# pallgeuer/novic

Measured on NVIDIA B200. Metric: labels/sec (greedy, batch 4096), higher is better.
Workload: dtype bf16

## Files before the change

include/novic_b200.h:

```cpp
#ifndef NOVIC_B200_H_
#define NOVIC_B200_H_

#include <stddef.h>
#include <stdint.h>

#ifdef __cplusplus
extern "C" {
#endif

#define NOVIC_MAX_LAYERS 16
#define NOVIC_MAX_BEAMS 16

typedef struct NovicCfg {
  int32_t embed_dim;
  int32_t hidden_dim;
  int32_t ffn_dim;
  int32_t num_layers;
  int32_t num_heads;
  int32_t prefix_len;
  int32_t vocab_size;
  int32_t token_length;
  int32_t strictly_causal;
  int32_t num_end_loss;
  float ln_eps;
// ... 157 lines not shown
  const float* proj_w[NOVIC_VIT_MAX_LAYERS];
  const float* proj_b[NOVIC_VIT_MAX_LAYERS];
  const float* norm2_w[NOVIC_VIT_MAX_LAYERS];
  const float* norm2_b[NOVIC_VIT_MAX_LAYERS];
  const float* fc1_w[NOVIC_VIT_MAX_LAYERS];
  const float* fc1_b[NOVIC_VIT_MAX_LAYERS];
  const float* fc2_w[NOVIC_VIT_MAX_LAYERS];
  const float* fc2_b[NOVIC_VIT_MAX_LAYERS];
} NovicSiglipWeights;
int novic_siglip_create(const NovicSiglipCfg* cfg, NovicVitHandle** out);
int novic_siglip_set_weights(NovicVitHandle* h, const NovicSiglipWeights* w, void* wbuf, size_t wbuf_bytes, void* stream);

int novic_debug_gemm(const void* a_bf16, const void* w_bf16, float* out, int32_t M, int32_t N, int32_t K,
                     int32_t block_n, void* stream);

int novic_debug_transpose_bf16(const void* src, int64_t rows, int32_t cols, int32_t ld_src, void* dst, int32_t ld_dst, void* stream);
int novic_debug_wgrad(const void* a_t, int32_t Mo, const void* b_t, int32_t No, int64_t K, int32_t ld, float* dw, void* stream);
int novic_debug_wgrad_mn(const void* a, int32_t Mo, int32_t ld_a, const void* b, int32_t No, int32_t ld_b, int64_t K, float* dw, void* stream);
int32_t novic_debug_wgrad_splits(int64_t tiles, int64_t kblocks, int32_t sms);

int novic_debug_vit_gemm(const void* a, const void* w, int32_t M, int32_t N, int32_t K, int32_t epi, int32_t act, int32_t direct, const float* bias,
                         void* dst, int32_t ld, const float* table, int32_t patches, int32_t tok0, int32_t path, int32_t grid_div, void* stream);
int novic_debug_vit_attention(const void* qkv, int32_t nimg, int32_t T, int32_t W, int32_t heads, int32_t kernel, int32_t max_ctas, void* out, void* stream);
int novic_debug_siglip_map_attention(const void* kv, const float* q, int32_t nimg, int32_t T, int32_t W, int32_t heads, void* out, void* stream);
int novic_debug_vit_layernorm(float* x, int64_t in_stride, const float* w1, const float* b1, const float* w2, const float* b2, int32_t store_x, void* out_bf,
                              int32_t rows, int32_t W, float eps, const float* cls, const float* pos0, int32_t cls_period, void* stream);

int novic_kernel_timing(int32_t enable);
int novic_kernel_times(double* ms_out, int64_t* count_out, int32_t n_classes);

// ... 20 lines not shown
```

novic_b200/_abi.py:

```python
from __future__ import annotations

import ctypes as C
import os
import subprocess

NOVIC_MAX_LAYERS = 16
NOVIC_MAX_BEAMS = 16

_HERE = os.path.dirname(os.path.abspath(__file__))
LIB_PATH = os.path.join(_HERE, "lib", "libnovic_b200.so")
CSRC_DIR = os.path.join(_HERE, "csrc")


class NovicCfg(C.Structure):
    _fields_ = [
        ("embed_dim", C.c_int32), ("hidden_dim", C.c_int32), ("ffn_dim", C.c_int32), ("num_layers", C.c_int32),
        ("num_heads", C.c_int32), ("prefix_len", C.c_int32), ("vocab_size", C.c_int32), ("token_length", C.c_int32),
        ("strictly_causal", C.c_int32), ("num_end_loss", C.c_int32), ("ln_eps", C.c_float), ("label_smoothing", C.c_float),
    ]


_FP = C.c_void_p


# ... 78 lines not shown
                                         C.c_void_p, C.c_size_t, C.c_void_p, C.c_int32, C.c_void_p]),
    "novic_adamw_scratch_bytes": (C.c_size_t, []),
    "novic_adamw_step": (C.c_int, [C.POINTER(NovicAdamW), _FP, _FP, _FP, _FP, C.c_int64, _FP, _FP, C.c_void_p, C.c_size_t, _FP, C.c_void_p]),
    "novic_vit_create": (C.c_int, [C.POINTER(NovicVitCfg), C.POINTER(C.c_void_p)]),
    "novic_vit_destroy": (C.c_int, [C.c_void_p]),
    "novic_vit_weight_bytes": (C.c_size_t, [C.c_void_p]),
    "novic_vit_set_weights": (C.c_int, [C.c_void_p, C.POINTER(NovicVitWeights), C.c_void_p, C.c_size_t, C.c_void_p]),
    "novic_vit_workspace_bytes": (C.c_size_t, [C.c_void_p, C.c_int64]),
    "novic_vit_encode": (C.c_int, [C.c_void_p, _FP, C.c_int64, _FP, C.c_int32, C.c_int64, C.c_void_p, C.c_size_t, C.c_void_p]),
    "novic_siglip_create": (C.c_int, [C.POINTER(NovicSiglipCfg), C.POINTER(C.c_void_p)]),
    "novic_siglip_set_weights": (C.c_int, [C.c_void_p, C.POINTER(NovicSiglipWeights), C.c_void_p, C.c_size_t, C.c_void_p]),
    "novic_set_dropout": (C.c_int, [C.c_void_p, C.c_float, C.c_float, C.c_uint64]),
    "novic_noise_apply": (C.c_int, [C.POINTER(NovicNoiseCfg), _FP, C.c_int64, C.c_uint64, C.c_uint64, C.c_void_p]),
    "novic_noise_apply_predrawn": (C.c_int, [C.POINTER(NovicNoiseCfg), _FP, C.c_int64, _FP, _FP, _FP, _FP, C.c_void_p]),
    "novic_debug_gemm": (C.c_int, [_FP, _FP, _FP, C.c_int32, C.c_int32, C.c_int32, C.c_int32, C.c_void_p]),
    "novic_debug_trace": (C.c_int, [C.POINTER(C.c_int64), C.c_int32]),
    "novic_debug_ws_offset": (C.c_int, [C.c_void_p, C.c_int64, C.c_int32, C.c_int32, C.c_char_p, C.POINTER(C.c_size_t)]),
    "novic_debug_keep_classes": (C.c_int, [C.c_void_p, C.c_uint32]),
    "novic_debug_redzone": (C.c_int, [C.c_size_t]),
    "novic_debug_zones": (C.c_int64, [C.c_void_p, C.c_int32, C.c_int64, C.c_int32, C.c_int32, C.POINTER(C.c_uint64), C.c_int64]),
    "novic_debug_transpose_bf16": (C.c_int, [_FP, C.c_int64, C.c_int32, C.c_int32, _FP, C.c_int32, C.c_void_p]),
    "novic_debug_wgrad": (C.c_int, [_FP, C.c_int32, _FP, C.c_int32, C.c_int64, C.c_int32, _FP, C.c_void_p]),
    "novic_debug_wgrad_mn": (C.c_int, [_FP, C.c_int32, C.c_int32, _FP, C.c_int32, C.c_int32, C.c_int64, _FP, C.c_void_p]),
    "novic_debug_wgrad_splits": (C.c_int32, [C.c_int64, C.c_int64, C.c_int32]),
    "novic_debug_vit_gemm": (C.c_int, [_FP, _FP, C.c_int32, C.c_int32, C.c_int32, C.c_int32, C.c_int32, C.c_int32, _FP, _FP, C.c_int32, _FP,
                                       C.c_int32, C.c_int32, C.c_int32, C.c_int32, C.c_void_p]),
    "novic_debug_vit_attention": (C.c_int, [_FP, C.c_int32, C.c_int32, C.c_int32, C.c_int32, C.c_int32, C.c_int32, _FP, C.c_void_p]),
    "novic_debug_siglip_map_attention": (C.c_int, [_FP, _FP, C.c_int32, C.c_int32, C.c_int32, C.c_int32, _FP, C.c_void_p]),
    "novic_debug_vit_layernorm": (C.c_int, [_FP, C.c_int64, _FP, _FP, _FP, _FP, C.c_int32, _FP, C.c_int32, C.c_int32, C.c_float, _FP, _FP, C.c_int32,
                                            C.c_void_p]),
# ... 47 lines not shown
```

novic_b200/csrc/abi.cu:

```cuda
#include <cstdarg>
#include <cstdio>
#include <cstring>
#include <map>
#include <mutex>
#include <string>
#include <tuple>
#include <vector>

#include "../../include/novic_b200.h"
#include "train.cuh"
#include "optim.cuh"
#include "vit.cuh"
#include "blockrows.cuh"

using namespace novic;

namespace {

thread_local std::string g_err;
int64_t g_launches = 0;

int fail(const char* fmt, ...) {
  char buf[1024];
  va_list ap;
// ... 108 lines not shown
int make_tmap_3d(CUtensorMap* map, const void* base, const cuuint64_t (&dims)[3], const cuuint64_t (&strides)[2], const cuuint32_t (&box)[3]) {
  if (load_driver_entry()) return 1;
  if ((reinterpret_cast<uintptr_t>(base) & 15) != 0 || strides[0] % 16 != 0 || strides[1] % 16 != 0) return fail("TMA operand base / strides must be 16-byte aligned");
  if (box[0] * 2 != 128) return fail("128-byte swizzle needs a 64-element inner box");
  cuuint32_t estr[3] = {1, 1, 1};
  CUresult r = g_encode(map, CU_TENSOR_MAP_DATA_TYPE_BFLOAT16, 3, const_cast<void*>(base), dims, strides, box, estr, CU_TENSOR_MAP_INTERLEAVE_NONE,
                        CU_TENSOR_MAP_SWIZZLE_128B, CU_TENSOR_MAP_L2_PROMOTION_L2_256B, CU_TENSOR_MAP_FLOAT_OOB_FILL_NONE);
  if (r != CUDA_SUCCESS) return fail("cuTensorMapEncodeTiled (3-D) failed with CUresult %d", (int)r);
  return 0;
}

constexpr int kStagesQKV = 5, kStagesGelu = 5, kStagesRow = 4, kStagesLogits = 5;
int g_block_rows64_min = 148 * 32 + 1;
int g_vit_direct = 1;
int g_block_rows = 0;
int g_qkv_ws = 1;
bool g_wgrad_mn = true;
constexpr int kWideKbs = 2, kWideStages = 3;
int g_num_sms = 148;
int g_logits_bn = 256;
int g_grid_div = 1;
constexpr int kLogitBN = kTileN;

bool g_use_pdl = true;
int g_cur_class = 9;
unsigned g_skip_classes = 0;
template <class... KArgs, class... Args>
cudaError_t launch_k(void (*kernel)(KArgs...), dim3 grid, dim3 block, size_t smem, cudaStream_t s, Args&&... args) {
  if ((g_skip_classes >> g_cur_class) & 1u) return cudaSuccess;
  cudaLaunchConfig_t cfg{};
  cfg.gridDim = grid; cfg.blockDim = block; cfg.dynamicSmemBytes = smem; cfg.stream = s;
// ... 37 lines not shown
  CUDA_TRY(launch_k(gemm_kernel<Epi, STAGES, 1, kTileN, kEpiWarps, MN>, dim3(grid), dim3(kGemmThreads), gemm_persistent_smem_bytes(STAGES, 1, kTileN, kEpiWarps), s, ta, tb, M, n_tiles,
                    static_cast<int>(ceil_div(K, kBlockK)), k_splits, 0, ep));
  ++g_launches;
  CUDA_TRY(cudaGetLastError());
  return 0;
}

static_assert(kE == kWsKb * kBlockK, "the weight-stationary kernel holds the whole K = 512 weight tile");
template <class Epi>
int set_gemm_ws_attr() {
  static_assert(gemm_ws_smem_bytes() <= 227 * 1024, "weight-stationary GEMM does not fit in shared memory");
  CUDA_TRY(cudaFuncSetAttribute(gemm_ws_kernel<Epi>, cudaFuncAttributeMaxDynamicSharedMemorySize, gemm_ws_smem_bytes()));
  return 0;
}
template <class Epi>
int launch_gemm_ws(cudaStream_t s, const CUtensorMap& ta, const CUtensorMap& tb, int M, int N, const typename Epi::Params& ep, bool b_is_static) {
  const int n_tiles = static_cast<int>(ceil_div(N, kTileN));
  const int per_tile = std::max(1, std::min<int>(g_num_sms / g_grid_div / n_tiles, static_cast<int>(ceil_div(M, kBlockM))));
  CUDA_TRY(launch_k(gemm_ws_kernel<Epi>, dim3(static_cast<unsigned>(n_tiles * per_tile)), dim3(kGemmThreads), gemm_ws_smem_bytes(), s, ta, tb, M, n_tiles, b_is_static ? 1 : 0, ep));
  ++g_launches;
  CUDA_TRY(cudaGetLastError());
  return 0;
}

template <class Epi, int STAGES, int PN = 256>
int set_gemm2_attr() {
  static_assert(gemm2_smem_bytes(STAGES, PN) <= 227 * 1024, "pair GEMM pipeline does not fit in shared memory");
  CUDA_TRY(cudaFuncSetAttribute(gemm2_kernel<Epi, STAGES, PN>, cudaFuncAttributeMaxDynamicSharedMemorySize, gemm2_smem_bytes(STAGES, PN)));
  return 0;
}
template <class Epi, int STAGES, int PN = 256>
int launch_gemm2(cudaStream_t s, const CUtensorMap& ta, const CUtensorMap& tb, int M, int N, int K, const typename Epi::Params& ep, bool b_is_static = false) {
  const int n_tiles = static_cast<int>(ceil_div(N, PN));
  const int64_t total = n_tiles * ceil_div(M, 2 * kBlockM);
// ... 322 lines not shown
  CUtensorMap tm_ao, tm_xn3, tm_ao32, tm_ao64r, tm_x_st;
  if (make_tmap(&tm_ao, ws.ao, M, kE, kBlockM)) return 1;
  if (make_tmap3(&tm_xn3, ws.xn, M, kE, kBlockM, kWideKbs)) return 1;
  if (make_tmap3(&tm_ao32, ws.ao, M, kE, kBrRows, kE / kBlockK)) return 1;
  if (make_tmap3(&tm_ao64r, ws.ao, M, kE, kB64Rows, kE / kBlockK)) return 1;
  if (make_tmap_xblk(&tm_x_st, ws.x, static_cast<int64_t>(ceil_div(M, 32)) * 32)) return 1;
  const bool rows64 = g_block_rows64_min > 0 && M >= g_block_rows64_min;
  const size_t kv_layer = static_cast<size_t>(ws.nseq) * S * kE;
  for (int l = 0; l < L; ++l) {
    {
      __nv_bfloat16* kc = ws.kv + (static_cast<size_t>(l) * 2 + 0) * kv_layer;
      __nv_bfloat16* vc = ws.kv + (static_cast<size_t>(l) * 2 + 1) * kv_layer;
      const EpiQKV::Params pq{ws.q, kc, vc, pc.nq, pc.q0, pc.slot_mul, S, 0};
      KSpan t(kKQkv, s);
      if (g_qkv_ws) {
        if (launch_gemm_ws<EpiQKV>(s, tm_xn3, h->w.tm_in_proj3[l], M, 3 * kE, pq, true)) return 1;
      } else if (launch_gemm<EpiQKV, kWideStages, kWideKbs>(s, tm_xn3, h->w.tm_in_proj3[l], M, 3 * kE, kE, pq, 1, true)) return 1;
    }
    if (launch_attention(h, ws, pc, l, s)) return 1;
    FusedBlockParams fb{};
    fb.x = ws.x; fb.gain_mid = h->w.norm2[l]; fb.eps = c.ln_eps;
    if (l + 1 < L) {
      fb.xn = ws.xn; fb.gain_out = h->w.norm1[l + 1];
    } else {
      fb.gain_out = h->w.final_norm;
      fb.xn = pc.remap_in > 0 ? ws.xfin : ws.xn;
      fb.remap_rows_in = pc.remap_in; fb.remap_skip = pc.remap_skip; fb.remap_rows_out = pc.remap_out;
    }
    KSpan t(kKFfn2, s);
    if (g_block_rows == 128) {
      if (launch_outproj_ffn(s, tm_ao, h->w.tm_out_proj[l], h->w.tm_linear1_q[l], h->w.tm_linear2[l], M, fb)) return 1;
// ... 233 lines not shown
  if (cfg->hidden_dim != kE) return fail("hidden_dim must be %d (got %d)", kE, cfg->hidden_dim);
  if (cfg->num_heads != kHeads) return fail("num_heads must be %d (got %d)", kHeads, cfg->num_heads);
  if (cfg->ffn_dim != 128) return fail("ffn_dim must be 128 (got %d)", cfg->ffn_dim);
  if (cfg->num_layers < 1 || cfg->num_layers > NOVIC_MAX_LAYERS) return fail("num_layers out of range");
  if (cfg->embed_dim % 128 != 0) return fail("embed_dim must be a multiple of 128 (got %d)", cfg->embed_dim);
  if (cfg->prefix_len < 1 || cfg->token_length < 2 || cfg->vocab_size < 2) return fail("bad prefix_len / token_length / vocab_size");
  if (cfg->prefix_len + cfg->token_length - 1 > 255) return fail("sequence too long");
  int dev = 0, n = 0;
  if (cudaGetDeviceCount(&n) != cudaSuccess || n == 0) return fail("no CUDA device: novic_b200 has no CPU fallback");
  CUDA_TRY(cudaGetDevice(&dev));
  cudaDeviceProp prop;
  CUDA_TRY(cudaGetDeviceProperties(&prop, dev));
  if (prop.major != 10) return fail("device %d is sm_%d%d; novic_b200 kernels are sm_100a only", dev, prop.major, prop.minor);
  if (load_driver_entry()) return 1;
  if (set_gemm_attr<EpiQKV, kStagesQKV>() || set_rowln_attr() || set_gemm_attr<EpiLogits<0>, kStagesLogits>() ||
      set_gemm_attr<EpiQKV, kWideStages, kWideKbs>() || set_gemm_ws_attr<EpiQKV>() || set_gemm_attr<EpiLogits<0>, 2, kWideKbs, 256, 16>() ||
      set_gemm_attr<EpiLogits<4>, 2, kWideKbs, 256, 16>() || set_gemm_attr<EpiLogits<12>, 2, kWideKbs, 256, 16>() ||
      set_gemm_attr<EpiLogits<4, true>, 2, kWideKbs, 256, 16>() || set_gemm_attr<EpiLogits<12, true>, 2, kWideKbs, 256, 16>() ||
      set_gemm_attr<EpiLogits<12>, kWideStages, kWideKbs>() || set_gemm_attr<EpiLogits<12, true>, kWideStages, kWideKbs>() ||
      set_gemm_attr<EpiLogits<12, true, true>, kWideStages, kWideKbs>() ||
      set_gemm_attr<EpiLogits<0>, kWideStages, kWideKbs>() || set_gemm_attr<EpiLogits<4>, kWideStages, kWideKbs>() ||
      set_gemm_attr<EpiLogits<16>, kWideStages, kWideKbs>() || set_gemm_attr<EpiLogits<0, true>, kWideStages, kWideKbs>() ||
      set_gemm_attr<EpiLogits<4, true>, kWideStages, kWideKbs>() || set_gemm_attr<EpiLogits<16, true>, kWideStages, kWideKbs>() ||
      set_gemm_attr<EpiLogits<4, true, true>, kWideStages, kWideKbs>() || set_gemm_attr<EpiLogits<16, true, true>, kWideStages, kWideKbs>() || set_gemm_attr<EpiStoreBF16, kStagesQKV>() || set_gemm_attr<EpiGeluTrain, kStagesGelu>() ||
      set_gemm_attr<EpiGradBlocked, kStagesQKV>() || set_gemm_attr<EpiAtomicF32, kStagesQKV>() || set_gemm_mn_attr<EpiAtomicF32, kStagesQKV>() || set_gemm_mn_attr<EpiGradBlocked, kStagesQKV, 2>() || set_gemm_mn_attr<EpiStoreBF16, kStagesQKV, 2>() || set_gemm_attr<EpiDLogits, kStagesLogits>())
    return 1;
  CUDA_TRY(cudaFuncSetAttribute(attn_bwd_kernel, cudaFuncAttributeMaxDynamicSharedMemorySize, attn_bwd_smem_bytes(kAttnBwdMaxS)));
  if (g_wd_host == nullptr) {
    CUDA_TRY(cudaHostAlloc(&g_wd_host, sizeof(unsigned int), cudaHostAllocMapped));
    *g_wd_host = 0;
    unsigned int* dptr = nullptr;
// ... 5 lines not shown
  h->device = dev;
  CUDA_TRY(cudaStreamCreateWithFlags(&h->capture_stream, cudaStreamNonBlocking));
  CUDA_TRY(cudaMallocHost(&h->h_flags, sizeof(int) * 8 * (cfg->token_length + 2)));
  CUDA_TRY(cudaMalloc(&h->d_drop_seed, 16));
  CUDA_TRY(cudaMemset(h->d_drop_seed, 0, 16));
  if (const char* e20 = getenv("NOVIC_TRAIN_GRAPHS")) h->train_graphs = e20[0] != '0';
  h->num_sms = prop.multiProcessorCount;
  g_num_sms = prop.multiProcessorCount;
  h->attn_smem_budget = std::min<int>(200 * 1024, static_cast<int>(prop.sharedMemPerBlockOptin) - 8 * 1024);
  CUDA_TRY(cudaFuncSetAttribute(attention_bulk_kernel, cudaFuncAttributeMaxDynamicSharedMemorySize, h->attn_smem_budget + 1024));
  CUDA_TRY(cudaFuncSetAttribute(select_greedy_kernel, cudaFuncAttributeMaxDynamicSharedMemorySize, kSelSmemBytes));
  CUDA_TRY(cudaFuncSetAttribute(attention_stream_kernel_t<16, 3, 4>, cudaFuncAttributeMaxDynamicSharedMemorySize, as_smem_bytes(16, 3, 4)));
  CUDA_TRY(cudaFuncSetAttribute(attention_split_kernel, cudaFuncAttributeMaxDynamicSharedMemorySize, kSpSmemBytes));
  CUDA_TRY(cudaFuncSetAttribute(attention_prefix_kernel, cudaFuncAttributeMaxDynamicSharedMemorySize, kApSmemBytes));
  if (const char* e = getenv("NOVIC_LOGITS_BN")) g_logits_bn = atoi(e);
  if (const char* e = getenv("NOVIC_QKV_WS")) g_qkv_ws = atoi(e) != 0 ? 1 : 0;
  if (const char* e = getenv("NOVIC_WGRAD_MN")) g_wgrad_mn = atoi(e) != 0;
  if (const char* e = getenv("NOVIC_BLOCK_ROWS")) g_block_rows = atoi(e);
  if (const char* e = getenv("NOVIC_VIT_DIRECT")) g_vit_direct = atoi(e) != 0 ? 1 : 0;
  if (const char* e = getenv("NOVIC_BLOCK_ROWS64_MIN")) g_block_rows64_min = atoi(e);
  if (const char* e = getenv("NOVIC_SKIP_CLASSES")) g_skip_classes = static_cast<unsigned>(strtoul(e, nullptr, 0));
  if (const char* e = getenv("NOVIC_ATTN_EARLY")) h->attn_early = atoi(e);
  if (const char* e = getenv("NOVIC_NO_PDL")) g_use_pdl = e[0] != '1';
  const char* env = getenv("NOVIC_NO_GRAPHS");
  if (env != nullptr && env[0] == '1') h->use_graphs = false;
  *out = h;
  return 0;
}

int novic_destroy(NovicHandle* h) {
  if (h == nullptr) return 0;
// ... 719 lines not shown
  CUDA_TRY(cudaFreeAsync(part, s));
  return rc;
}

int32_t novic_debug_wgrad_splits(int64_t tiles, int64_t kblocks, int32_t sms) {
  if (tiles < 1 || kblocks < 1 || sms < 1) return -1;
  return choose_wgrad_splits(tiles, kblocks, sms);
}

int novic_debug_transpose_bf16(const void* src, int64_t rows, int32_t cols, int32_t ld_src, void* dst, int32_t ld_dst, void* stream) {
  if (rows < 1 || cols < 1 || ld_src < cols || ld_dst < rows) return fail("bad transpose shape");
  return launch_transpose(static_cast<cudaStream_t>(stream), static_cast<const __nv_bfloat16*>(src), rows, cols, ld_src,
                          static_cast<__nv_bfloat16*>(dst), ld_dst);
}

int novic_debug_wgrad_mn(const void* a, int32_t Mo, int32_t ld_a, const void* b, int32_t No, int32_t ld_b, int64_t K, float* dw, void* stream) {
  if (Mo < 1 || No < 1 || K < 1) return fail("bad wgrad shape");
  if (set_gemm_mn_attr<EpiAtomicF32, kStagesQKV>()) return 1;
  return launch_wgrad_mn(static_cast<cudaStream_t>(stream), static_cast<const __nv_bfloat16*>(a), Mo, ld_a, static_cast<const __nv_bfloat16*>(b), No, ld_b, K, dw);
}

int novic_debug_wgrad(const void* a_t, int32_t Mo, const void* b_t, int32_t No, int64_t K, int32_t ld, float* dw, void* stream) {
  if (Mo < 1 || No < 1 || K < 1 || ld < K || ld % 8 != 0) return fail("bad wgrad shape (ld must be a multiple of 8 and >= K)");
  if (set_gemm_attr<EpiAtomicF32, kStagesQKV>()) return 1;
  return launch_wgrad(static_cast<cudaStream_t>(stream), static_cast<const __nv_bfloat16*>(a_t), Mo, static_cast<const __nv_bfloat16*>(b_t), No, K, ld, dw);
}

}

#include "vit_host.inc"
// ... 1 lines not shown
```

novic_b200/csrc/gemm.cuh:

```cuda
#pragma once

#include "ptx.cuh"

namespace novic {

constexpr int kE = 512;
constexpr int kBlockM = 128;
constexpr int kBlockK = 64;
constexpr int kUmmaK = 16;
constexpr int kTileN = 128;
constexpr int kABytes = kBlockM * kBlockK * 2;
constexpr int kBBytes = kTileN * kBlockK * 2;
constexpr int kStageBytes = kABytes + kBBytes;
constexpr int kStagePitch = kTileN * 2 + 16;
constexpr int kWarpStageBytes = 32 * kStagePitch;

__host__ __device__ __forceinline__ size_t xblk_off(int row, int col4) {
  return ((static_cast<size_t>(row >> 5) * (kE / 4) + col4) * 32 + (row & 31)) * 4;
}

__host__ __device__ constexpr int gemm_smem_bytes(int stages) { return stages * kStageBytes + 1024  + 256  + 1536 ; }

struct EpiCtx {
  uint32_t tmem_row;
// ... 39 lines not shown
      else *reinterpret_cast<uint4*>(dst + chunk * 8) = v;
    }
  }
  __syncwarp();
}


struct EpiQKV {
  struct Params {
    __nv_bfloat16* q;
    __nv_bfloat16* kcache;
    __nv_bfloat16* vcache;
    int rows_per_seq, pos0, slot_mul, smax;
    int kv_hint;
  };
  template <class Release>
  __device__ static __forceinline__ void run(const Params& p, const EpiCtx& c, Release release) {
    const int lane = lane_id();
    const int nparts = c.ncols / kEpiCols;
    if (c.stage == nullptr) {
      for (int part = 0; part < nparts; ++part) {
        const int n0 = c.n0 + part * kEpiCols;
        __nv_bfloat16* dst = nullptr;
        if (c.row < c.M) {
          if (n0 < kE) dst = p.q + static_cast<size_t>(c.row) * kE + n0;
          else {
            const int seq = c.row / p.rows_per_seq;
            const int pos = p.pos0 + (c.row - seq * p.rows_per_seq);
            const size_t page = (static_cast<size_t>(seq) * p.slot_mul * p.smax + pos) * kE;
            dst = (n0 < 2 * kE) ? p.kcache + page + (n0 - kE) : p.vcache + page + (n0 - 2 * kE);
          }
        }
#pragma unroll
        for (int ch = 0; ch < kEpiCols / 32; ++ch) {
          float v[32];
          tmem_ld_32x32(c.tmem_row + part * kEpiCols + ch * 32, v);
          if (part == nparts - 1 && ch == kEpiCols / 32 - 1) release();
          if (dst != nullptr) {
#pragma unroll
            for (int h = 0; h < 2; ++h) {
              uint32_t w[8];
#pragma unroll
              for (int i = 0; i < 8; ++i) w[i] = pack_bf16x2(v[h * 16 + 2 * i], v[h * 16 + 2 * i + 1]);
              asm volatile("st.global.v8.b32 [%0], {%1, %2, %3, %4, %5, %6, %7, %8};\n" ::"l"(dst + ch * 32 + h * 16), "r"(w[0]), "r"(w[1]), "r"(w[2]),
                           "r"(w[3]), "r"(w[4]), "r"(w[5]), "r"(w[6]), "r"(w[7])
                           : "memory");
            }
// ... 1 lines not shown
        }
      }
      return;
    }
    for (int part = 0; part < nparts; ++part) {
#pragma unroll
      for (int ch = 0; ch < kEpiCols / 32; ++ch) {
        float v[32];
        tmem_ld_32x32(c.tmem_row + part * kEpiCols + ch * 32, v);
        if (part == nparts - 1 && ch == kEpiCols / 32 - 1) release();
        stage_put32(c.stage, lane, ch * 32, v);
      }
      const int n0 = c.n0 + part * kEpiCols;
      stage_copy_out(c.stage, lane, [&](int r) -> __nv_bfloat16* {
        const int row = c.warp_row0 + r;
        if (row >= c.M) return nullptr;
        if (n0 < kE) return p.q + static_cast<size_t>(row) * kE + n0;
        const int seq = row / p.rows_per_seq;
        const int pos = p.pos0 + (row - seq * p.rows_per_seq);
        const size_t page = (static_cast<size_t>(seq) * p.slot_mul * p.smax + pos) * kE;
        return (n0 < 2 * kE) ? p.kcache + page + (n0 - kE) : p.vcache + page + (n0 - 2 * kE);
      }, (n0 >= kE && p.kv_hint) ? kEvictLast : 0ull);
    }
  }
};

__device__ __forceinline__ float gelu_fast(float x) {
  const float ax = fabsf(x) * 0.70710678118654752440f;
  const float t = __fdividef(1.0f, fmaf(0.3275911f, ax, 1.0f));
  float poly = fmaf(t, 1.061405429f, -1.453152027f);
  poly = fmaf(poly, t, 1.421413741f);
  poly = fmaf(poly, t, -0.284496736f);
  poly = fmaf(poly, t, 0.254829592f);
  const float erf_abs = 1.0f - poly * t * __expf(-ax * ax);
  return 0.5f * x * (1.0f + copysignf(erf_abs, x));
}
// ... 569 lines not shown
      Epi::run(ep, c, [rel, lane]() {
        tc_fence_before_sync();
        __syncwarp();
        if (lane == 0) mbar_arrive(rel);
      });
      if (i < 8 && threadIdx.x == 64) trace_point(tr, 17 + 2 * i);
    }
  }

  tc_fence_before_sync();
  __syncthreads();
  if (threadIdx.x == 0) trace_point(tr, 10);
  if (warp == 1) tmem_dealloc<kAccStages * kTileN>(tmem_base);
}

constexpr int kRowBN = kTileN;
constexpr int kRowCluster = kE / kRowBN;
constexpr int kRowEpiWarps = 8;
constexpr int kRowThreads = 64 + 32 * kRowEpiWarps;
constexpr int kRowCols = kRowBN / 2;
constexpr int kRowStagePitch = kRowCols * 2 + 16;
constexpr int kFfnDim = 128;

struct RowParams {
  float* x;
  const float* x_in;
  __nv_bfloat16* xn;
  const float* gain;
  const float* pos;
  int prefix_rep;
// ... 784 lines not shown
```

novic_b200/csrc/ptx.cuh:

```cuda
#pragma once

#include <cstdint>
#include <cuda.h>
#include <cuda_bf16.h>
#include <cuda_runtime.h>

namespace novic {

__device__ __forceinline__ uint32_t smem_u32(const void* p) {
  return static_cast<uint32_t>(__cvta_generic_to_shared(p));
}

__device__ __forceinline__ uint32_t lane_id() { return threadIdx.x & 31u; }

__device__ __forceinline__ bool elect_one() {
  uint32_t pred;
  asm volatile(
      "{\n\t.reg .pred p;\n\t"
      "elect.sync _|p, 0xffffffff;\n\t"
      "selp.u32 %0, 1, 0, p;\n\t}\n"
      : "=r"(pred));
  return pred != 0;
}

// ... 202 lines not shown
         | (0u << 16)
         | ((N >> 3) << 17)
         | ((M >> 4) << 24);
}

__device__ __forceinline__ void umma_bf16_ss(uint32_t tmem_d, uint64_t desc_a, uint64_t desc_b, uint32_t idesc,
                                             uint32_t accumulate) {
  asm volatile(
      "{\n\t.reg .pred p;\n\t"
      "setp.ne.b32 p, %4, 0;\n\t"
      "tcgen05.mma.cta_group::1.kind::f16 [%0], %1, %2, %3, p;\n\t}\n" ::"r"(tmem_d),
      "l"(desc_a), "l"(desc_b), "r"(idesc), "r"(accumulate)
      : "memory");
}

__device__ __forceinline__ void umma_commit(uint64_t* bar) {
  asm volatile("tcgen05.commit.cta_group::1.mbarrier::arrive::one.shared::cluster.b64 [%0];\n" ::"r"(smem_u32(bar))
               : "memory");
}

template <uint32_t kCols>
__device__ __forceinline__ void tmem_alloc2(uint32_t* smem_dst) {
  static_assert(kCols >= 32 && kCols <= 512 && (kCols & (kCols - 1)) == 0, "TMEM columns: power of two in [32,512]");
  asm volatile("tcgen05.alloc.cta_group::2.sync.aligned.shared::cta.b32 [%0], %1;\n" ::"r"(smem_u32(smem_dst)), "n"(kCols) : "memory");
  asm volatile("tcgen05.relinquish_alloc_permit.cta_group::2.sync.aligned;\n" ::: "memory");
}
template <uint32_t kCols>
__device__ __forceinline__ void tmem_dealloc2(uint32_t taddr) {
  asm volatile("tcgen05.dealloc.cta_group::2.sync.aligned.b32 %0, %1;\n" ::"r"(taddr), "n"(kCols) : "memory");
}
// ... 152 lines not shown
```

novic_b200/csrc/train_host.inc:

```

struct TrainLayerBufs {
  float* x_in;
  float* x_mid;
  __nv_bfloat16* xn1;
  __nv_bfloat16* q;
  __nv_bfloat16* k;
  __nv_bfloat16* v;
  __nv_bfloat16* ao;
  __nv_bfloat16* xn2;
  __nv_bfloat16* hpre;
  __nv_bfloat16* h;
};

struct TrainPlan {
  int64_t B = 0, A = 0, R = 0, Rt = 0;
  int M = 1, C = 0, S = 0, ldR = 0, ldRt = 0, ldB = 0, Vp = 0, nparts = 0;
  bool has_pad = false;
  TrainLayerBufs layer[NOVIC_MAX_LAYERS];
  float* ein; __nv_bfloat16* ebf; __nv_bfloat16* ebf_t;
  float* x_last;
  __nv_bfloat16* xfin;
  __nv_bfloat16* xfin_t;
  LogitPartial* part; float* lse; float* nll_rows; float* loss; unsigned char* correct;
  unsigned char* keypad; unsigned char* effpad; long long* tgt_masked; float* row_weight;
// ... 139 lines not shown
  if (din.thresh != 0u) {
    input_dropout_ln_kernel<<<static_cast<unsigned>(ceil_div(static_cast<int64_t>(R), 4)), 128, 0, s>>>(t.layer[0].x_in, t.layer[0].xn1, h->w.norm1[0], R, c.ln_eps,
                                                                                                       din, site(0, kDropInput));
    ++g_launches;
  }
  for (int l = 0; l < L; ++l) {
    const TrainLayerBufs& lb = t.layer[l];
    CUtensorMap tm_xn1, tm_ao, tm_xn2, tm_h;
    if (make_tmap(&tm_xn1, lb.xn1, R, kE, kBlockM) || make_tmap(&tm_ao, lb.ao, R, kE, kBlockM) || make_tmap(&tm_xn2, lb.xn2, R, kE, kBlockM) ||
        make_tmap(&tm_h, lb.h, R, c.ffn_dim, kBlockM))
      return 1;
    EpiQKV::Params pq{lb.q, lb.k, lb.v, S, 0, 1, smax, 0};
    if (g_qkv_ws && ceil_div(R, kBlockM) >= 2 * (g_num_sms / (3 * kE / kTileN))) {
      CUtensorMap tm_xn1w;
      if (make_tmap3(&tm_xn1w, lb.xn1, R, kE, kBlockM, kWideKbs)) return 1;
      if (launch_gemm_ws<EpiQKV>(s, tm_xn1w, h->w.tm_in_proj3[l], static_cast<int>(R), 3 * kE, pq, true)) return 1;
    } else if (launch_gemm<EpiQKV, kStagesQKV>(s, tm_xn1, h->w.tm_in_proj[l], R, 3 * kE, kE, pq)) return 1;
    AttnParams pa{};
    pa.q = lb.q; pa.kcache = lb.k; pa.vcache = lb.v; pa.out = lb.ao; pa.keypad = has_pad ? t.keypad : nullptr; pa.anc = nullptr;
    pa.nseq = A; pa.nq = S; pa.q0 = 0; pa.smax = smax; pa.P = P; pa.beams = 1; pa.slot_mul = 1;
    pa.prefix_bidir = c.strictly_causal ? 0 : 1; pa.keypad_ld = S; pa.anc_ld = 0;
    pa.scale_log2e = 1.4426950408889634f / sqrtf(static_cast<float>(kHeadDim));
    pa.drop = dl; pa.drop_site = site(l, kDropAttn);
    {
      const unsigned grid = static_cast<unsigned>(ceil_div(static_cast<int64_t>(A) * kHeads, kAttnTfWarps));
      if (dl.thresh != 0u) attention_tf_kernel<true><<<grid, kAttnTfWarps * 32, kAttnTfSmemBytes, s>>>(pa);
      else attention_tf_kernel<false><<<grid, kAttnTfWarps * 32, kAttnTfSmemBytes, s>>>(pa);
      CUDA_TRY(cudaGetLastError());
      ++g_launches;
    }
    RowParams po{};
// ... 160 lines not shown
```

Before: 844,300.

## Add weight-stationary QKV GEMM keeping the weight tile in TMEM

```diff
diff --git a/include/novic_b200.h b/include/novic_b200.h
--- a/include/novic_b200.h
+++ b/include/novic_b200.h
@@ -195,6 +195,9 @@
 int novic_debug_gemm(const void* a_bf16, const void* w_bf16, float* out, int32_t M, int32_t N, int32_t K,
                      int32_t block_n, void* stream);
 
+int novic_debug_qkv_gemm(const void* x, const void* w, int32_t M, void* q, void* kcache, void* vcache, int32_t rows_per_seq, int32_t pos0,
+                         int32_t slot_mul, int32_t smax, int32_t impl, void* stream);
+
 int novic_debug_transpose_bf16(const void* src, int64_t rows, int32_t cols, int32_t ld_src, void* dst, int32_t ld_dst, void* stream);
 int novic_debug_wgrad(const void* a_t, int32_t Mo, const void* b_t, int32_t No, int64_t K, int32_t ld, float* dw, void* stream);
 int novic_debug_wgrad_mn(const void* a, int32_t Mo, int32_t ld_a, const void* b, int32_t No, int32_t ld_b, int64_t K, float* dw, void* stream);
diff --git a/novic_b200/_abi.py b/novic_b200/_abi.py
--- a/novic_b200/_abi.py
+++ b/novic_b200/_abi.py
@@ -116,6 +116,7 @@
     "novic_noise_apply": (C.c_int, [C.POINTER(NovicNoiseCfg), _FP, C.c_int64, C.c_uint64, C.c_uint64, C.c_void_p]),
     "novic_noise_apply_predrawn": (C.c_int, [C.POINTER(NovicNoiseCfg), _FP, C.c_int64, _FP, _FP, _FP, _FP, C.c_void_p]),
     "novic_debug_gemm": (C.c_int, [_FP, _FP, _FP, C.c_int32, C.c_int32, C.c_int32, C.c_int32, C.c_void_p]),
+    "novic_debug_qkv_gemm": (C.c_int, [_FP, _FP, C.c_int32, _FP, _FP, _FP, C.c_int32, C.c_int32, C.c_int32, C.c_int32, C.c_int32, C.c_void_p]),
     "novic_debug_trace": (C.c_int, [C.POINTER(C.c_int64), C.c_int32]),
     "novic_debug_ws_offset": (C.c_int, [C.c_void_p, C.c_int64, C.c_int32, C.c_int32, C.c_char_p, C.POINTER(C.c_size_t)]),
     "novic_debug_keep_classes": (C.c_int, [C.c_void_p, C.c_uint32]),
diff --git a/novic_b200/csrc/abi.cu b/novic_b200/csrc/abi.cu
--- a/novic_b200/csrc/abi.cu
+++ b/novic_b200/csrc/abi.cu
@@ -146,7 +146,7 @@
 int g_block_rows64_min = 148 * 32 + 1;
 int g_vit_direct = 1;
 int g_block_rows = 0;
-int g_qkv_ws = 1;
+int g_qkv_ws = 2;
 bool g_wgrad_mn = true;
 constexpr int kWideKbs = 2, kWideStages = 3;
 int g_num_sms = 148;
@@ -214,10 +214,19 @@
   return 0;
 }
 template <class Epi>
-int launch_gemm_ws(cudaStream_t s, const CUtensorMap& ta, const CUtensorMap& tb, int M, int N, const typename Epi::Params& ep, bool b_is_static) {
+int set_gemm_wst_attr() {
+  static_assert(gemm_wst_smem_bytes() <= 227 * 1024, "weight-stationary TMEM GEMM does not fit in shared memory");
+  CUDA_TRY(cudaFuncSetAttribute(gemm_wst_kernel<Epi>, cudaFuncAttributeMaxDynamicSharedMemorySize, gemm_wst_smem_bytes()));
+  return 0;
+}
+template <class Epi>
+int launch_gemm_ws(cudaStream_t s, const CUtensorMap& ta, const CUtensorMap& tb, int M, int N, const typename Epi::Params& ep, bool b_is_static,
+                   bool tmem_a) {
   const int n_tiles = static_cast<int>(ceil_div(N, kTileN));
   const int per_tile = std::max(1, std::min<int>(g_num_sms / g_grid_div / n_tiles, static_cast<int>(ceil_div(M, kBlockM))));
-  CUDA_TRY(launch_k(gemm_ws_kernel<Epi>, dim3(static_cast<unsigned>(n_tiles * per_tile)), dim3(kGemmThreads), gemm_ws_smem_bytes(), s, ta, tb, M, n_tiles, b_is_static ? 1 : 0, ep));
+  const dim3 grid(static_cast<unsigned>(n_tiles * per_tile));
+  if (tmem_a) CUDA_TRY(launch_k(gemm_wst_kernel<Epi>, grid, dim3(kGemmThreads), gemm_wst_smem_bytes(), s, ta, tb, M, n_tiles, b_is_static ? 1 : 0, ep));
+  else CUDA_TRY(launch_k(gemm_ws_kernel<Epi>, grid, dim3(kGemmThreads), gemm_ws_smem_bytes(), s, ta, tb, M, n_tiles, b_is_static ? 1 : 0, ep));
   ++g_launches;
   CUDA_TRY(cudaGetLastError());
   return 0;
@@ -570,7 +579,7 @@
       const EpiQKV::Params pq{ws.q, kc, vc, pc.nq, pc.q0, pc.slot_mul, S, 0};
       KSpan t(kKQkv, s);
       if (g_qkv_ws) {
-        if (launch_gemm_ws<EpiQKV>(s, tm_xn3, h->w.tm_in_proj3[l], M, 3 * kE, pq, true)) return 1;
+        if (launch_gemm_ws<EpiQKV>(s, tm_xn3, h->w.tm_in_proj3[l], M, 3 * kE, pq, true, g_qkv_ws == 2)) return 1;
       } else if (launch_gemm<EpiQKV, kWideStages, kWideKbs>(s, tm_xn3, h->w.tm_in_proj3[l], M, 3 * kE, kE, pq, 1, true)) return 1;
     }
     if (launch_attention(h, ws, pc, l, s)) return 1;
@@ -834,7 +843,7 @@
   if (prop.major != 10) return fail("device %d is sm_%d%d; novic_b200 kernels are sm_100a only", dev, prop.major, prop.minor);
   if (load_driver_entry()) return 1;
   if (set_gemm_attr<EpiQKV, kStagesQKV>() || set_rowln_attr() || set_gemm_attr<EpiLogits<0>, kStagesLogits>() ||
-      set_gemm_attr<EpiQKV, kWideStages, kWideKbs>() || set_gemm_ws_attr<EpiQKV>() || set_gemm_attr<EpiLogits<0>, 2, kWideKbs, 256, 16>() ||
+      set_gemm_attr<EpiQKV, kWideStages, kWideKbs>() || set_gemm_ws_attr<EpiQKV>() || set_gemm_wst_attr<EpiQKV>() || set_gemm_attr<EpiLogits<0>, 2, kWideKbs, 256, 16>() ||
       set_gemm_attr<EpiLogits<4>, 2, kWideKbs, 256, 16>() || set_gemm_attr<EpiLogits<12>, 2, kWideKbs, 256, 16>() ||
       set_gemm_attr<EpiLogits<4, true>, 2, kWideKbs, 256, 16>() || set_gemm_attr<EpiLogits<12, true>, 2, kWideKbs, 256, 16>() ||
       set_gemm_attr<EpiLogits<12>, kWideStages, kWideKbs>() || set_gemm_attr<EpiLogits<12, true>, kWideStages, kWideKbs>() ||
@@ -870,7 +879,8 @@
   CUDA_TRY(cudaFuncSetAttribute(attention_split_kernel, cudaFuncAttributeMaxDynamicSharedMemorySize, kSpSmemBytes));
   CUDA_TRY(cudaFuncSetAttribute(attention_prefix_kernel, cudaFuncAttributeMaxDynamicSharedMemorySize, kApSmemBytes));
   if (const char* e = getenv("NOVIC_LOGITS_BN")) g_logits_bn = atoi(e);
-  if (const char* e = getenv("NOVIC_QKV_WS")) g_qkv_ws = atoi(e) != 0 ? 1 : 0;
+  if (const char* e = getenv("NOVIC_QKV_WS")) g_qkv_ws = std::max(0, std::min(2, atoi(e)));
+  else g_qkv_ws = 2;
   if (const char* e = getenv("NOVIC_WGRAD_MN")) g_wgrad_mn = atoi(e) != 0;
   if (const char* e = getenv("NOVIC_BLOCK_ROWS")) g_block_rows = atoi(e);
   if (const char* e = getenv("NOVIC_VIT_DIRECT")) g_vit_direct = atoi(e) != 0 ? 1 : 0;
@@ -1620,6 +1630,19 @@
                           static_cast<__nv_bfloat16*>(dst), ld_dst);
 }
 
+int novic_debug_qkv_gemm(const void* x, const void* w, int32_t M, void* q, void* kcache, void* vcache, int32_t rows_per_seq, int32_t pos0,
+                         int32_t slot_mul, int32_t smax, int32_t impl, void* stream) {
+  if (M < 1 || rows_per_seq < 1 || pos0 < 0 || slot_mul < 1 || pos0 + rows_per_seq > smax) return fail("bad QKV projection shape");
+  if (impl < 0 || impl > 2) return fail("impl must be 0 (generic kernel), 1 (weight tile in shared memory) or 2 (weight tile in TMEM)");
+  cudaStream_t s = static_cast<cudaStream_t>(stream);
+  CUtensorMap ta, tb;
+  if (make_tmap3(&ta, x, M, kE, kBlockM, kWideKbs) || make_tmap3(&tb, w, 3 * kE, kE, kTileN, kWideKbs)) return 1;
+  const EpiQKV::Params p{static_cast<__nv_bfloat16*>(q), static_cast<__nv_bfloat16*>(kcache), static_cast<__nv_bfloat16*>(vcache), rows_per_seq, pos0,
+                         slot_mul, smax, 0};
+  if (impl == 0) return set_gemm_attr<EpiQKV, kWideStages, kWideKbs>() || launch_gemm<EpiQKV, kWideStages, kWideKbs>(s, ta, tb, M, 3 * kE, kE, p, 1, true);
+  return set_gemm_ws_attr<EpiQKV>() || set_gemm_wst_attr<EpiQKV>() || launch_gemm_ws<EpiQKV>(s, ta, tb, M, 3 * kE, p, true, impl == 2);
+}
+
 int novic_debug_wgrad_mn(const void* a, int32_t Mo, int32_t ld_a, const void* b, int32_t No, int32_t ld_b, int64_t K, float* dw, void* stream) {
   if (Mo < 1 || No < 1 || K < 1) return fail("bad wgrad shape");
   if (set_gemm_mn_attr<EpiAtomicF32, kStagesQKV>()) return 1;
diff --git a/novic_b200/csrc/gemm.cuh b/novic_b200/csrc/gemm.cuh
--- a/novic_b200/csrc/gemm.cuh
+++ b/novic_b200/csrc/gemm.cuh
@@ -77,6 +77,41 @@
     int rows_per_seq, pos0, slot_mul, smax;
     int kv_hint;
   };
+  __device__ static __forceinline__ __nv_bfloat16* out_at(const Params& p, int row, int n0) {
+    if (n0 < kE) return p.q + static_cast<size_t>(row) * kE + n0;
+    const int seq = row / p.rows_per_seq;
+    const int pos = p.pos0 + (row - seq * p.rows_per_seq);
+    const size_t page = (static_cast<size_t>(seq) * p.slot_mul * p.smax + pos) * kE;
+    return (n0 < 2 * kE) ? p.kcache + page + (n0 - kE) : p.vcache + page + (n0 - 2 * kE);
+  }
+
+  template <class Release>
+  __device__ static __forceinline__ void run_transposed(const Params& p, const EpiCtx& c, Release release) {
+    const int lane = lane_id();
+    const int r = lane >> 1, cq = (lane & 1) * 2;
+#pragma unroll
+    for (int ch = 0; ch < 2; ++ch) {
+      float v[32];
+      tmem_ld_32x32(c.tmem_row + ch * 32, v);
+      if (ch == 1) release();
+#pragma unroll
+      for (int j = 0; j < 32; ++j)
+        *reinterpret_cast<__nv_bfloat16*>(c.stage + j * 64 + (((lane >> 3) ^ ((j >> 1) & 1)) << 4) + (lane & 7) * 2) = __float2bfloat16_rn(v[j]);
+      __syncwarp();
+#pragma unroll
+      for (int h = 0; h < 2; ++h) {
+        const int rs = r + 16 * h;
+        const uint4 lo = *reinterpret_cast<const uint4*>(c.stage + rs * 64 + ((cq ^ ((rs >> 1) & 1)) << 4));
+        const uint4 hi = *reinterpret_cast<const uint4*>(c.stage + rs * 64 + (((cq + 1) ^ ((rs >> 1) & 1)) << 4));
+        const int row = c.warp_row0 + ch * 32 + rs;
+        if (row < c.M)
+          asm volatile("st.global.v8.b32 [%0], {%1, %2, %3, %4, %5, %6, %7, %8};\n" ::"l"(out_at(p, row, c.n0) + (lane & 1) * 16), "r"(lo.x), "r"(lo.y),
+                       "r"(lo.z), "r"(lo.w), "r"(hi.x), "r"(hi.y), "r"(hi.z), "r"(hi.w)
+                       : "memory");
+      }
+      __syncwarp();
+    }
+  }
   template <class Release>
   __device__ static __forceinline__ void run(const Params& p, const EpiCtx& c, Release release) {
     const int lane = lane_id();
@@ -85,15 +120,7 @@
       for (int part = 0; part < nparts; ++part) {
         const int n0 = c.n0 + part * kEpiCols;
         __nv_bfloat16* dst = nullptr;
-        if (c.row < c.M) {
-          if (n0 < kE) dst = p.q + static_cast<size_t>(c.row) * kE + n0;
-          else {
-            const int seq = c.row / p.rows_per_seq;
-            const int pos = p.pos0 + (c.row - seq * p.rows_per_seq);
-            const size_t page = (static_cast<size_t>(seq) * p.slot_mul * p.smax + pos) * kE;
-            dst = (n0 < 2 * kE) ? p.kcache + page + (n0 - kE) : p.vcache + page + (n0 - 2 * kE);
-          }
-        }
+        if (c.row < c.M) dst = out_at(p, c.row, n0);
 #pragma unroll
         for (int ch = 0; ch < kEpiCols / 32; ++ch) {
           float v[32];
@@ -125,12 +152,7 @@
       const int n0 = c.n0 + part * kEpiCols;
       stage_copy_out(c.stage, lane, [&](int r) -> __nv_bfloat16* {
         const int row = c.warp_row0 + r;
-        if (row >= c.M) return nullptr;
-        if (n0 < kE) return p.q + static_cast<size_t>(row) * kE + n0;
-        const int seq = row / p.rows_per_seq;
-        const int pos = p.pos0 + (row - seq * p.rows_per_seq);
-        const size_t page = (static_cast<size_t>(seq) * p.slot_mul * p.smax + pos) * kE;
-        return (n0 < 2 * kE) ? p.kcache + page + (n0 - kE) : p.vcache + page + (n0 - 2 * kE);
+        return row < c.M ? out_at(p, row, n0) : nullptr;
       }, (n0 >= kE && p.kv_hint) ? kEvictLast : 0ull);
     }
   }
@@ -730,6 +752,154 @@
   if (warp == 1) tmem_dealloc<kAccStages * kTileN>(tmem_base);
 }
 
+constexpr int kWstStages = 6;
+constexpr int kWstWeightStage0 = 2;
+constexpr int kWstAccCol0 = kWsKb * kBlockK / 2;
+constexpr int kWstEpiBytes = 32 * 32 * 2;
+__host__ __device__ constexpr int gemm_wst_smem_bytes() { return kWstStages * kWsABytes + kEpiWarps * kWstEpiBytes + 1024 + 256; }
+
+template <class Epi>
+__global__ void __launch_bounds__(kGemmThreads, 1)
+gemm_wst_kernel(const __grid_constant__ CUtensorMap tmap_a, const __grid_constant__ CUtensorMap tmap_b, int M, int n_tiles, int b_is_static,
+                typename Epi::Params ep) {
+  static_assert(kWstStages - kWstWeightStage0 == kWsKb / 2, "the weight tile fills the ring's last four stages");
+  extern __shared__ uint8_t smem_raw[];
+  uint8_t* smem = reinterpret_cast<uint8_t*>((reinterpret_cast<uintptr_t>(smem_raw) + 1023) & ~uintptr_t(1023));
+  uint8_t* ring = smem;
+  uint8_t* epi_smem = ring + kWstStages * kWsABytes;
+  uint64_t* b_full = reinterpret_cast<uint64_t*>(epi_smem + kEpiWarps * kWstEpiBytes);
+  uint64_t* b_free = b_full + kWsKb / 2;
+  uint64_t* a_full = b_free + 1;
+  uint64_t* a_empty = a_full + kWstStages;
+  uint64_t* tmem_full_bar = a_empty + kWstStages;
+  uint64_t* tmem_empty_bar = tmem_full_bar + kAccStages;
+  uint32_t* tmem_slot = reinterpret_cast<uint32_t*>(tmem_empty_bar + kAccStages);
+  __shared__ int s_trace;
+
+  const int warp = threadIdx.x >> 5;
+  const int m_blocks = (M + kBlockM - 1) / kBlockM;
+  const int nt = blockIdx.x % n_tiles, g0 = blockIdx.x / n_tiles, gstep = gridDim.x / n_tiles;
+  const int n0 = nt * kTileN;
+  pdl_trigger();
+  if (threadIdx.x == 0) { s_trace = trace_begin() ? 1 : 0; trace_point(s_trace != 0, 0); }
+
+  auto load_weights = [&]() {
+    for (int j = 0; j < kWsKb / 2; ++j) {
+      mbar_arrive_expect_tx(&b_full[j], kWsABytes);
+      tma_load_3d(ring + (kWstWeightStage0 + j) * kWsABytes, &tmap_b, &b_full[j], n0, 2 * j, kEvictLast);
+    }
+  };
+  if (warp == 0) {
+    if (elect_one()) {
+      tma_prefetch_desc(&tmap_a);
+      tma_prefetch_desc(&tmap_b);
+      for (int j = 0; j < kWsKb / 2; ++j) mbar_init(&b_full[j], 1);
+      mbar_init(b_free, 1);
+      for (int s = 0; s < kWstStages; ++s) { mbar_init(&a_full[s], 1); mbar_init(&a_empty[s], 1); }
+      for (int a = 0; a < kAccStages; ++a) { mbar_init(&tmem_full_bar[a], 1); mbar_init(&tmem_empty_bar[a], kEpiWarps); }
+      fence_mbar_init();
+      if (b_is_static && g0 < m_blocks) load_weights();
+    }
+  } else if (warp == 1) {
+    tmem_alloc<kWstAccCol0 + kAccStages * kTileN>(tmem_slot);
+  }
+  tc_fence_before_sync();
+  __syncthreads();
+  tc_fence_after_sync();
+  const uint32_t tmem_base = *tmem_slot;
+  const bool tr = s_trace != 0;
+  pdl_wait();
+  if (threadIdx.x == 0) trace_point(tr, 1);
+
+  if (warp == 0) {
+    if (elect_one()) {
+      if (!b_is_static && g0 < m_blocks) load_weights();
+      int stage = 0; uint32_t phase = 0;
+      for (int mb = g0; mb < m_blocks; mb += gstep) {
+        for (int j = 0; j < kWsKb / 2; ++j) {
+          if (phase == 0 && stage >= kWstWeightStage0) mbar_wait(b_free, 0, 12);
+          mbar_wait(&a_empty[stage], phase ^ 1, 1);
+          mbar_arrive_expect_tx(&a_full[stage], kWsABytes);
+          tma_load_3d(ring + stage * kWsABytes, &tmap_a, &a_full[stage], mb * kBlockM, 2 * j, kEvictNormal);
+          if (++stage == kWstStages) { stage = 0; phase ^= 1; }
+        }
+      }
+      trace_point(tr, 3);
+    }
+  } else if (warp == 1) {
+    if (elect_one()) {
+      constexpr uint32_t kIdesc = umma_idesc_bf16_f32(kBlockM, kTileN);
+      if (g0 < m_blocks) {
+        for (int j = 0; j < kWsKb / 2; ++j) {
+          mbar_wait(&b_full[j], 0, 4);
+          tc_fence_after_sync();
+          const uint32_t sb = smem_u32(ring + (kWstWeightStage0 + j) * kWsABytes);
+#pragma unroll
+          for (int s = 0; s < 2 * kBlockK / kUmmaK; ++s)
+            tmem_cp_128x256b(tmem_base + (j * 2 * kBlockK / kUmmaK + s) * 8, umma_desc_sw128_kmajor(sb + (s >> 2) * kBBytes + (s & 3) * (kUmmaK * 2)));
+        }
+        umma_commit(b_free);
+        mbar_wait(b_free, 0, 13);
+        tc_fence_after_sync();
+      }
+      int stage = 0; uint32_t phase = 0;
+      int i = 0;
+      for (int mb = g0; mb < m_blocks; mb += gstep, ++i) {
+        const int as = i & 1;
+        mbar_wait(&tmem_empty_bar[as], ((i >> 1) & 1) ^ 1, 9);
+        tc_fence_after_sync();
+        const uint32_t acc = tmem_base + kWstAccCol0 + as * kTileN;
+        for (int j = 0; j < kWsKb / 2; ++j) {
+          mbar_wait(&a_full[stage], phase, 2);
+          if (i == 0 && j == 0) trace_point(tr, 4);
+          tc_fence_after_sync();
+          const uint32_t sa = smem_u32(ring + stage * kWsABytes);
+#pragma unroll
+          for (int jj = 0; jj < 2; ++jj)
+#pragma unroll
+            for (int k = 0; k < kBlockK / kUmmaK; ++k)
+              umma_bf16_ts(acc, tmem_base + ((2 * j + jj) * (kBlockK / kUmmaK) + k) * 8, umma_desc_sw128_kmajor(sa + jj * kABytes + k * (kUmmaK * 2)),
+                           kIdesc, (j | jj | k) != 0 ? 1u : 0u);
+          umma_commit(&a_empty[stage]);
+          if (++stage == kWstStages) { stage = 0; phase ^= 1; }
+        }
+        umma_commit(&tmem_full_bar[as]);
+        if (i == 0) trace_point(tr, 5);
+      }
+    }
+  } else {
+    const int ew = warp - 2;
+    const int quad = warp & 3;
+    const int half = ew >> 2;
+    const int lane = static_cast<int>(lane_id());
+    int i = 0;
+    for (int mb = g0; mb < m_blocks; mb += gstep, ++i) {
+      const int as = i & 1;
+      mbar_wait(&tmem_full_bar[as], (i >> 1) & 1, 3);
+      if (i < 8 && threadIdx.x == 64) trace_point(tr, 16 + 2 * i);
+      tc_fence_after_sync();
+      EpiCtx c;
+      c.tmem_row = tmem_base + (static_cast<uint32_t>(quad * 32) << 16) + kWstAccCol0 + as * kTileN + half * (kBlockM / 2);
+      c.warp_row0 = mb * kBlockM + half * (kBlockM / 2);
+      c.n0 = n0 + quad * 32;
+      c.M = M;
+      c.stage = epi_smem + ew * kWstEpiBytes;
+      uint64_t* rel = &tmem_empty_bar[as];
+      Epi::run_transposed(ep, c, [rel, lane]() {
+        tc_fence_before_sync();
+        __syncwarp();
+        if (lane == 0) mbar_arrive(rel);
+      });
+      if (i < 8 && threadIdx.x == 64) trace_point(tr, 17 + 2 * i);
+    }
+  }
+
+  tc_fence_before_sync();
+  __syncthreads();
+  if (threadIdx.x == 0) trace_point(tr, 10);
+  if (warp == 1) tmem_dealloc<kWstAccCol0 + kAccStages * kTileN>(tmem_base);
+}
+
 constexpr int kRowBN = kTileN;
 constexpr int kRowCluster = kE / kRowBN;
 constexpr int kRowEpiWarps = 8;
diff --git a/novic_b200/csrc/ptx.cuh b/novic_b200/csrc/ptx.cuh
--- a/novic_b200/csrc/ptx.cuh
+++ b/novic_b200/csrc/ptx.cuh
@@ -240,6 +240,19 @@
       : "memory");
 }
 
+__device__ __forceinline__ void umma_bf16_ts(uint32_t tmem_d, uint32_t tmem_a, uint64_t desc_b, uint32_t idesc, uint32_t accumulate) {
+  asm volatile(
+      "{\n\t.reg .pred p;\n\t"
+      "setp.ne.b32 p, %4, 0;\n\t"
+      "tcgen05.mma.cta_group::1.kind::f16 [%0], [%1], %2, %3, p;\n\t}\n" ::"r"(tmem_d),
+      "r"(tmem_a), "l"(desc_b), "r"(idesc), "r"(accumulate)
+      : "memory");
+}
+
+__device__ __forceinline__ void tmem_cp_128x256b(uint32_t taddr, uint64_t desc) {
+  asm volatile("tcgen05.cp.cta_group::1.128x256b [%0], %1;\n" ::"r"(taddr), "l"(desc) : "memory");
+}
+
 __device__ __forceinline__ void umma_commit(uint64_t* bar) {
   asm volatile("tcgen05.commit.cta_group::1.mbarrier::arrive::one.shared::cluster.b64 [%0];\n" ::"r"(smem_u32(bar))
                : "memory");
diff --git a/novic_b200/csrc/train_host.inc b/novic_b200/csrc/train_host.inc
--- a/novic_b200/csrc/train_host.inc
+++ b/novic_b200/csrc/train_host.inc
@@ -177,7 +177,7 @@
     if (g_qkv_ws && ceil_div(R, kBlockM) >= 2 * (g_num_sms / (3 * kE / kTileN))) {
       CUtensorMap tm_xn1w;
       if (make_tmap3(&tm_xn1w, lb.xn1, R, kE, kBlockM, kWideKbs)) return 1;
-      if (launch_gemm_ws<EpiQKV>(s, tm_xn1w, h->w.tm_in_proj3[l], static_cast<int>(R), 3 * kE, pq, true)) return 1;
+      if (launch_gemm_ws<EpiQKV>(s, tm_xn1w, h->w.tm_in_proj3[l], static_cast<int>(R), 3 * kE, pq, true, g_qkv_ws == 2)) return 1;
     } else if (launch_gemm<EpiQKV, kStagesQKV>(s, tm_xn1, h->w.tm_in_proj[l], R, 3 * kE, kE, pq)) return 1;
     AttnParams pa{};
     pa.q = lb.q; pa.kcache = lb.k; pa.vcache = lb.v; pa.out = lb.ao; pa.keypad = has_pad ? t.keypad : nullptr; pa.anc = nullptr;
```

Result: faster. 853,100, median of 6 (+1.0%).
